# bioinformatics-centre/BayesTyper

Measured on AMD Instinct MI355X. Metric: variant-cluster Gibbs iterations/sec + k-mer matches/sec at 1/2/4/8 MI355X, higher is better.
Workload: dtype f64 log-probabilities over u8 k-mer counts (Gibbs); u64/u8 integer (k-mer matching)

## Files before the change

### bayestyper_amd/csrc/bt_gibbs.hip

```cpp
#ifndef BT_SWEEP_OUTLINE
#define BT_SWEEP_INLINE
#endif
#include "bt_genotypes.hpp"
#include "bt_gibbs_kernel.hpp"
#include "bt_gibbs_timeline.hpp"
#include "bt_internal.hpp"

#include <algorithm>
#include <atomic>
#include <chrono>
#include <cmath>
#include <cstring>
#include <map>
#include <memory>
#include <numeric>

using namespace bt;

namespace bt {
hipError_t launch_gibbs_simple_kernel(unsigned grid, uint32_t lds, hipStream_t st, const TileDesc *tiles, uint8_t *pool, const GParams *P, int op, uint32_t a0, uint32_t a1,
                                      unsigned long long *hist, TraceCfg tr, const uint32_t *tile_list, TimelineDev *tl);
hipError_t prepare_gibbs_simple_kernel(int max_lds);
hipError_t launch_gibbs_hot_kernel(unsigned grid, unsigned block, uint32_t lds, hipStream_t st, const TileDesc *tiles, uint8_t *pool, const GParams *P, int op, uint32_t a0, uint32_t a1,
                                   unsigned long long *hist, TraceCfg tr, const uint32_t *tile_list, TimelineDev *tl);
// ... 818 lines not shown
            BT_HIP(launch_gibbs_hot_kernel(c.pack_wgs, LANES * c.pack_waves, c.pack_lds, st, g->d_tiles, g->d_pool, g->d_params, op, a0, a1, hist, tr, (const uint32_t *)c.d_pack, tl));
        else if (tl)
            hipLaunchKernelGGL(gibbs_kernel_tl, dim3((unsigned)c.tiles.size()), dim3(LANES * c.split), c.lds, st, g->d_tiles, g->d_pool, g->d_params, op, a0, a1, hist, tr,
                               (const uint32_t *)c.d_tiles, tl);
        else
            hipLaunchKernelGGL(gibbs_kernel, dim3((unsigned)c.tiles.size()), dim3(LANES * c.split), c.lds, st, g->d_tiles, g->d_pool, g->d_params, op, a0, a1, hist, tr,
                               (const uint32_t *)c.d_tiles);
        BT_CHECK_LAUNCH();
        if (tl) tl += class_waves(c);
        if (wide && c.num_fill) {
            hipLaunchKernelGGL(nan_fill_kernel, dim3(c.num_fill), dim3(256), 0, st, g->d_pool, (const FillChunk *)c.d_fill);
            BT_CHECK_LAUNCH();
        }
        if (c.stream) BT_HIP(hipEventRecord(c.done, st));
    }
    for (auto &c : g->classes)
        if (c.stream) BT_HIP(hipStreamWaitEvent(g->ctx->stream, c.done, 0));
    g->prefill_armed = wide;
    return BT_OK;
}

inline uint64_t align_up(uint64_t x, uint64_t a) { return (x + a - 1) / a * a; }
inline uint32_t tile_lds_bytes(const TileDesc &d) { return d.lds_all ? d.hot_bytes * d.nvm : d.hot_bytes; }
constexpr uint32_t kBulkSubsetDefault = 1;
constexpr uint32_t kMinTileWidth = 4;
constexpr uint32_t kLightLds = 24576;
const uint32_t kClassLds[] = {16384, 32768, 0xFFFFFFFFu};

const uint32_t kElemSize[A_COUNT] = {
     1,  1,  1,  1,  4,  4,  2,  4,  2,  4,  4,  4,  2,
     1,  4,  4,  4,  2,  4,  4,  4,  4,  4,  4,
     4,  1,
     4,  8,  8,  4,  4,  4,  4,  1,  2,  8,  4,  1,
     4,  4,  4,  4,  4,  4,  8,  4,  8,  2,  8,
     8,  4,  8,  1,  4,  4,  8,  1,  1,  8,  4,  8,  4,  1,  4,  8,  4,
     4,  1,  8,  4,  4,  4,  1,  1,  1,  1,  4,  2,  4,  8,  8,  4,  2,  1,  4,  4,  4,  1,  1,  1,  1,  4,  4};

}

extern "C" {

struct bt_gibbs_source {
    bt_ctx *ctx = nullptr;
    uint32_t S = 0, G = 0, C = 0;
    std::vector<ClusterDims> cd;
    std::vector<GroupDims> gd;
// ... 330 lines not shown
        C = (uint32_t)cd_sel.size();
        cd = cd_sel.data();
        gd = gd_sel.data();
    }
    if (G == 0 || C == 0) return fail("bt_gibbs_create: empty batch");
    BT_HIP(hipSetDevice(ctx->device));
    bt_gibbs *g = new bt_gibbs();
    g->ctx = ctx;
    g->G = G;
    g->C = C;
    g->S = S;
    GParams &P = g->P;
    P.S = S;
    P.seed = params->seed;
    P.num_chains = params->num_chains;
    P.burn_in = params->burn_in;
    P.num_iterations = params->num_iterations;
    P.max_hvk = params->max_haplotype_variant_kmers;
    P.noise_seeding = params->noise_seeding;
    P.rate = (double)params->kmer_subsampling_rate;
    {
        const char *e = getenv("BT_GIBBS_BULK_SUBSET");
        P.bulk_subset = e ? (atoi(e) != 0 ? 1u : 0u) : kBulkSubsetDefault;
    }
    for (uint32_t s = 0; s < S; ++s) P.gender[s] = params->gender[s] ? 1 : 0;

#define BT_TRY(x)                \
    do {                         \
        int _rc = (x);           \
        if (_rc != BT_OK) {      \
            bt_gibbs_destroy(g); \
            return _rc;          \
        }                        \
    } while (0)
#define BT_TRYHIP(x)                                                     \
    do {                                                                 \
        hipError_t _e = (x);                                             \
        if (_e != hipSuccess) {                                          \
            bt_gibbs_destroy(g);                                         \
            return fail(std::string(#x) + ": " + hipGetErrorString(_e)); \
        }                                                                \
    } while (0)

    g->h_A.assign(C, 0);
    g->h_var_off.assign((size_t)C + 1, 0);
    for (uint32_t c = 0; c < C; ++c) g->h_var_off[c + 1] = g->h_var_off[c] + cd[c].V;
// ... 2097 lines not shown
```

### bayestyper_amd/csrc/bt_gibbs_tile.hpp

```cpp
#pragma once
#include "bt_rng_device.hpp"

namespace bt {

constexpr unsigned LANES = 64;
constexpr uint16_t NOHAP = 0xFFFF;
constexpr double BT_LN2 = 0.693147180559945309417232121458176568;
constexpr double BT_DBL_EPS = 2.220446049250313080847263336181640625e-16;
#ifndef BT_LINEAR_DRAW_MIN
#define BT_LINEAR_DRAW_MIN 4u
#endif
#ifndef BT_UC_INVALIDATE_MIN
#define BT_UC_INVALIDATE_MIN 64u
#endif
#ifndef BT_EVAL_BLOCK
#define BT_EVAL_BLOCK 4u
#endif
constexpr uint32_t EVB = BT_EVAL_BLOCK;
#ifdef BT_SINGLE
constexpr bool kSingle = true;
#else
constexpr bool kSingle = false;
#endif
#ifdef BT_PACKED
// ... 121 lines not shown
    uint32_t teams;
    uint32_t sblk;
};
#ifndef BT_EV_CAP
#define BT_EV_CAP 32
#endif
constexpr uint32_t EV_CAP = BT_EV_CAP;
constexpr uint32_t KSC_WAYS = 4;
constexpr uint32_t KSC_NOKEY = 0xFFFEFFFEu;
constexpr uint32_t NOHOT = 0xFFFFFFFFu;
constexpr uint32_t RESIDENT_ALL = 0xFFFFFFFEu;
constexpr uint32_t RESIDENT_NEVER = 0xFFFFFFFDu;

struct GParams {
    uint32_t S, seed, num_chains, burn_in, num_iterations, max_hvk, noise_seeding;
    double rate;
    uint8_t gender[32];
    const double BT_GAS *lut_g;
    const double BT_GAS *lut_n;
    const double BT_GAS *lgamma_int;
    const double BT_GAS *gamma_a2;
    uint32_t lgamma_n, gamma_n;
    uint32_t bulk_subset;
};

extern __shared__ __attribute__((aligned(16))) uint8_t bt_lds_raw[];
__device__ inline uint8_t *lds_block() { return (uint8_t *)bt_lds_raw; }
__device__ inline uint32_t pack_slot() { return blockIdx.x * (blockDim.x >> 6) + (uint32_t)__builtin_amdgcn_readfirstlane((int)(threadIdx.x >> 6)); }

__host__ __device__ constexpr bool hot_core(int a) {
    return a == A_SC || a == A_DIP || a == A_NESTPL || a == A_NESTN || a == A_KSCUPD || a == A_PEND || a == A_PENDDIP || a == A_PENDVALID || a == A_EVN || a == A_FREQ || a == A_LOGF ||
           a == A_OBS || a == A_NZ || a == A_NZLIST || a == A_UNEXT || a == A_ZHDR || a == A_ZBKT || a == A_PHDR || a == A_PBKT || a == A_RING || a == A_FNDSAVED;
}

struct Tile {
    uint8_t BT_GAS *base;
    const TileDesc BT_CAS *d;
    uint32_t lane;
    uint32_t plane;
    uint32_t part, copies;
    uint32_t wsh;
    uint8_t *hot;
    uint32_t lds0;
    uint32_t resident;
    template <typename T>
    __device__ inline SPtrF<T, LANES> harr(int a, uint32_t v, uint32_t len) const {
// ... 314 lines not shown
__device__ inline double count_log_prob(const GParams BT_CAS &P, uint32_t s, uint8_t mult, uint8_t count) {
    if (mult == 0) return P.lut_n[s * 256u + count];
    return P.lut_g[((uint32_t)s * 256u + mult) * 256u + count];
}

__device__ inline uint8_t dip_mult(const Vx &c, uint32_t k, uint16_t h1, uint16_t h2) {
    uint8_t m = 0;
    if (h1 != NOHAP) m = (uint8_t)(m + c.M(k, h1));
    if (h2 != NOHAP) m = (uint8_t)(m + c.M(k, h2));
    return m;
}
__device__ inline uint8_t unique_mult(const Vx &c, uint32_t k, uint16_t h1, uint16_t h2, uint8_t gender) {
    uint8_t m = dip_mult(c, k, h1, h2);
    if (c.has_counts(k)) m = (uint8_t)(m + c.ic(k, gender));
    return m;
}
__device__ inline uint8_t multi_mult(const Vx &c, const GParams BT_CAS &P, uint32_t k, uint16_t h1, uint16_t h2, uint16_t p1, uint16_t p2, uint32_t s) {
    const uint8_t icm = c.ic(k, P.gender[s]);
    if (c.count(k, s) == 0) return (uint8_t)(dip_mult(c, k, h1, h2) + icm);
    const uint8_t shared = c.shared_mult()[(uint32_t)c.shared_idx(k) * P.S + s];
    return (uint8_t)(shared - dip_mult(c, k, p1, p2) + dip_mult(c, k, h1, h2) + icm);
}

__device__ inline void freq_reset(const Vx &c) {
    const double f = 1 / (double)c.H;
    const double lf = bt_log(f);
    SPtrF<uint32_t, LANES> obs = c.obs();
    SPtrF<double, LANES> freq = c.freq(), logf = c.logf();
    SPtrF<uint8_t, LANES> nz = c.nz();
    for (uint32_t h = 0; h < c.H; ++h) {
        obs[h] = 0;
        freq[h] = f;
        logf[h] = lf;
        nz[h] = 1;
    }
    if (c.sc()[SC_IS_SPARSE]) {
        uset_clear(c.plus_set());
        Vx::HSet z = c.zero_set();
        uset_clear(z);
        for (uint32_t h = 0; h < c.H; ++h) uset_insert(z, h);
    }
}

template <class G>
__device__ inline uint32_t sparsity_cover(const Vx &c, G &rng) {
    TPtr<uint8_t> rows = c.cover_rows();
    SPtrF<uint32_t, LANES> obs = c.obs();
    SPtrF<uint16_t, LANES> nzl = c.nzlist();
    const uint32_t Hm = c.d().Hm, H = c.H;
// ... 85 lines not shown
        TPtr<uint32_t> dk = c.dip_keys(), df = c.dip_freq();
        for (uint32_t i = 0; i < d.dip_cap; ++i) dk[i] = 0;
        for (size_t i = 0; i < (uint32_t)d.dip_cap * P.S; ++i) df[i] = 0;
        TPtr<uint32_t> sl = c.sclen();
        for (uint32_t i = 0; i < d.scache_n; ++i) sl[i] = 0;
    }
    c.rng_seed(1, prng_seed);
    uint32_t cover;
    {
        MtRing m = c.rng(1);
        cover = sparsity_cover(c, m);
    }
    c.rng_seed(1, prng_seed);
    c.fnd_saved() = 0;
    sc[SC_FND_AVAIL] = 0;
    sc[SC_IS_SPARSE] = cover > 0 ? 1u : 0u;
    if (cover > 0) {
        const double sp = (double)cover / (double)c.H;
        const double cap = 1 - BT_DBL_EPS * 100;
        c.sparsity() = sp < cap ? sp : cap;
        uset_init(c.zero_set());
        uset_init(c.plus_set());
    }
    freq_reset(c);
    sc[SC_CONSTRUCTED] = 1;
}

__device__ inline uint32_t hashed_slot(const Vx &c, uint32_t key) {
    const uint32_t sub = c.d().cache_entries / c.t.copies;
    return ((key * 2654435761u) & (sub - 1u)) + c.t.part * sub;
}

__device__ inline bool wide_table(const TileDesc BT_CAS &d) { return d.cache_mode == 0 && !d.simple && d.cache_entries > BT_UC_INVALIDATE_MIN && d.hoff[A_UCACHE] == NOHOT; }

__device__ inline void cache_clear(const Vx &c, const GParams BT_CAS &P, bool all_copies_run, bool wide_fill = false) {
    const TileDesc BT_CAS &d = c.d();
    if (wide_fill && !all_copies_run && wide_table(d)) {
        c.sc()[SC_UC_DIRTY] = 0;
    } else if (d.cache_mode == 0) {
        c.sc()[SC_UC_DIRTY] = (!all_copies_run && d.cache_entries > BT_UC_INVALIDATE_MIN) ? 2u : 1u;
    } else if (d.cache_mode == 1) {
        TPtr<uint32_t> tg = c.uctag();
        const uint32_t sub = all_copies_run ? d.cache_entries / c.t.copies : d.cache_entries;
        for (uint32_t i = all_copies_run ? c.t.part * sub : 0u, e = i + sub; i < e; ++i) tg[i] = 0;
    }
    if (!kSingle && d.NMm) {
        SPtrF<uint32_t, LANES> mg = c.mgen();
// ... 172 lines not shown
    sc[SC_NSUB_U] = nsu;
    sc[SC_NSUB_M] = nsm;
    TPtr<uint8_t> smm = c.smm(), oth = c.oth();
    for (uint32_t i = bulk ? c.t.part : 0u, step = bulk ? c.t.copies : 1u; i < nsm * P.S; i += step) {
        smm[i] = 0;
        oth[i] = 0;
    }
    for (uint32_t s = 0; s < P.S; ++s) c.mgen()[s] += 1;
    SPtrF<uint8_t, LANES> upd = c.ksc_upd();
    for (uint32_t s = bulk ? c.t.part : 0u, step = bulk ? c.t.copies : 1u; s < P.S; s += step) {
        upd[s] = 1;
        for (uint32_t e = 0; e < KSC_WAYS; ++e) c.ksc_key(s)[e] = KSC_NOKEY;
        c.ksc_key(s)[KSC_WAYS] = 0;
    }
    if (bulk) copies_sync();
}

__device__ BT_NOINLINE void genotyper_reset(Env env, uint32_t vtx, bool bulk) {
    const Vx c = make_vx(make_tile(env), vtx);
    const GParams BT_CAS &P = env_params(env);
    c.sc()[SC_USE_MULTI] = 0;
    sample_kmer_subset(c, P, bulk);
    cache_clear(c, P, true);
    freq_reset(c);
}

__device__ inline uint32_t dip_index(const Vx &c, uint16_t h1, uint16_t h2) {
    if (h2 == NOHAP) return c.H * (c.H + 1) / 2 + h1;
    return (uint32_t)h1 * c.H - ((uint32_t)h1 * ((uint32_t)h1 - 1u)) / 2u + ((uint32_t)h2 - (uint32_t)h1);
}

__device__ inline double unique_log_prob(const Vx &c, const GParams BT_CAS &P, uint32_t s, uint16_t h1, uint16_t h2, uint32_t nsub_u) {
    const TileDesc BT_CAS &d = c.d();
    const uint32_t idx = dip_index(c, h1, h2);
    uint32_t slot = 0;
    const Vx::UCPtr uc = c.ucache();
    if (d.cache_mode == 0) {
        const double v = uc[(uint32_t)s * d.Dcm + idx];
        if (v == v) return v;
    } else if (d.cache_mode == 1) {
        const uint32_t key = s * d.Dcm + idx + 1u;
        slot = hashed_slot(c, key);
        if (c.uctag()[slot] == key) return uc[slot];
    }
    double acc = 0;
    const uint8_t gender = P.gender[s];
    {
// ... 649 lines not shown
                TPtr<double> pn = c.pend_nest(s);
                same = (double)pn[3] == (double)nn;
                for (uint32_t j = 0; j < 2u; ++j)
                    if (j < nn) {
                        TPtr<double> q = c.nest_stats(s, j);
                        same = same && (double)q[0] == (double)pn[4 * j] && (double)q[1] == (double)pn[4 * j + 1] && (double)q[2] == (double)pn[4 * j + 2];
                    }
            } else
                same = true;
            if (same) {
                c.pend()[s] += 1;
                continue;
            }
        }
#endif
#ifdef BT_COLLECT_OUTLINE
        collect_sample_slow(env, vtx, s);
#else
        collect_sample_body(c, P, s, nsub_u, nsub_m);
#endif
    }
}

__device__ BT_SWEEPFN void sample_diplotypes(Env env, uint32_t vtx, bool collect, uint32_t trace_word, bool tracing, uint32_t *trace_buf) {
    const Vx c = make_vx(make_tile(env), vtx);
    const GParams BT_CAS &P = env_params(env);
    const TPtr<uint32_t> trace_row{(uint32_t BT_GAS *)uniform_ptr(trace_buf), trace_word, 6u};
    SPtrF<uint32_t, LANES> sc = c.sc();
    const uint32_t nsub_u = sc[SC_NSUB_U], nsub_m = kSingle ? 0u : (uint32_t)sc[SC_NSUB_M];
    const bool use_multi = !kSingle && sc[SC_USE_MULTI] != 0, is_sparse = sc[SC_IS_SPARSE] != 0;
    uint32_t hap_count = sc[SC_HAP_COUNT];
    PROF_DECL;
    if (sc[SC_UC_DIRTY] == 2u) {
        const Vx::UCPtr ucl = c.ucache();
        const double nan = __builtin_nan("");
        for (uint32_t i = c.t.part, n = c.d().cache_entries; i < n; i += c.t.copies) ucl[i] = nan;
        if (c.t.copies > 1u) copies_sync();
        sc[SC_UC_DIRTY] = 0;
    } else if (sc[SC_UC_DIRTY]) {
        fill_unique_cache(env, vtx);
        sc[SC_UC_DIRTY] = 0;
    }
    PROF(12);
    MtRing rng = c.rng(0);
    SPtrF<uint16_t, LANES> nzl = c.nzlist();
    SPtrF<double, LANES> logf = c.logf();
    SPtrF<uint16_t, LANES> dip = c.dip();
    uint32_t nnz = 0;
    {
        SPtrF<uint8_t, LANES> nz = c.nz();
        for (uint32_t h = 0; h < c.H; ++h)
            if (nz[h]) nzl[nnz++] = (uint16_t)h;
    }
    PROF(0);
    const uint32_t T = c.t.copies > 1u && c.d().teams > 1u ? c.d().teams : 1u;
    const uint32_t tsz = c.t.copies / T, team = c.t.part / tsz, tpart = c.t.part - team * tsz;
    const uint32_t cw = 64u / c.t.copies, gl = (threadIdx.x & 63u) % cw, tlane0 = gl + team * tsz * cw;
    SPtrF<double, LANES> cum = c.cum() + (team < T ? team : 0u) * (c.d().D2m > 1 ? c.d().D2m : 1);
    for (uint32_t s0 = 0; s0 < P.S; s0 += T) {
      double u01 = 0;
      for (uint32_t j = 0; j < T && s0 + j < P.S; ++j) {
          const double u = rng_canonical(rng);
          if (j == team) u01 = u;
      }
      PROF(24);
      const uint32_t s = s0 + team;
      uint32_t mine = 0xFFFFFFFFu;
      if (team < T && s < P.S) {
        const uint16_t p1 = dip[2 * s], p2 = dip[2 * s + 1];
        const uint8_t ploidy = c.nest_ploidy()[s];
        uint32_t gen = 0;
        if (use_multi && nsub_m) {
            multi_refresh(c, P, s, p1, p2, nsub_m);
            gen = c.mgen()[s];
        }
        PROF(1);
        const uint32_t total = ploidy == 2 ? nnz * (nnz + 1) / 2 : (ploidy == 1 ? nnz : 0u);
        const bool chain_only = total <= BT_LINEAR_DRAW_MIN;
        const bool par = !chain_only && tsz > 1u;
        double lpmax = 0;
        auto eval_candidates = [&]() {
            const bool dipl = ploidy == 2;
            const TileDesc BT_CAS &dd = c.d();
            const Vx::UCPtr uc = c.ucache();
            TPtr<double> mc = c.mcache();
            TPtr<uint32_t> uct = c.uctag(), mct = c.mctag(), mcg = c.mcgen();
            const bool multi = use_multi && nsub_m != 0;
            uint32_t a = 0, b = 0;
            auto advance = [&](uint32_t steps) {
                if (!dipl) {
                    a += steps;
                    return;
                }
                while (steps > 0 && a < nnz) {
                    const uint32_t left = nnz - b;
                    if (steps < left) {
                        b += steps;
                        steps = 0;
                    } else {
                        steps -= left;
                        ++a;
                        b = a;
                    }
                }
// ... 9 lines not shown
                uint32_t utag[EVB], mtag[EVB], mgn[EVB];
#pragma unroll
                for (uint32_t q = 0; q < EVB; ++q) {
                    if (q < nb) {
                        ha[q] = nzl[a];
                        hb[q] = dipl ? (uint16_t)nzl[b] : NOHAP;
                        if (dipl) {
                            if (++b == nnz) {
                                ++a;
                                b = a;
                            }
                        } else
                            ++a;
                        const uint32_t idx = dip_index(c, ha[q], hb[q]);
                        ukey[q] = s * dd.Dcm + idx + 1u;
                        uslot[q] = dd.cache_mode == 0 ? s * dd.Dcm + idx : hashed_slot(c, ukey[q]);
                        uval[q] = dd.cache_mode != 2 ? (double)uc[uslot[q]] : 0.0;
                        utag[q] = dd.cache_mode == 1 ? (uint32_t)uct[uslot[q]] : 0u;
                        if (multi) {
                            mtag[q] = mct[uslot[q]];
                            mgn[q] = mcg[uslot[q]];
                            mval[q] = mc[uslot[q]];
                        }
                        la[q] = logf[ha[q]];
                        lb[q] = dipl ? (double)logf[hb[q]] : 0.0;
                    }
                }
                if (multi) {
                    bool need[EVB], any = false;
#pragma unroll
                    for (uint32_t q = 0; q < EVB; ++q) {
                        need[q] = q < nb && !(mtag[q] == ukey[q] && mgn[q] == gen);
                        any = any || need[q];
                    }
                    if (any) {
                        double fresh[EVB];
                        multi_log_prob_block(c, P, s, ha, hb, need, nsub_m, fresh);
#pragma unroll
                        for (uint32_t q = 0; q < EVB; ++q)
                            if (need[q]) {
                                mval[q] = fresh[q];
                                mct[uslot[q]] = ukey[q];
                                mcg[uslot[q]] = gen;
                                mc[uslot[q]] = fresh[q];
                            }
                    }
                }
                {
                    bool umiss[EVB], any = false;
#pragma unroll
                    for (uint32_t q = 0; q < EVB; ++q) {
                        umiss[q] = q < nb && !((dd.cache_mode == 0 && uval[q] == uval[q]) || (dd.cache_mode == 1 && utag[q] == ukey[q]));
                        any = any || umiss[q];
                    }
                    if (any) {
                        double fresh[EVB];
                        unique_log_prob_block(c, P, s, ha, hb, umiss, nsub_u, fresh);
#pragma unroll
                        for (uint32_t q = 0; q < EVB; ++q)
                            if (umiss[q]) uval[q] = fresh[q];
                    }
                }
#pragma unroll
                for (uint32_t q = 0; q < EVB; ++q) {
                    if (q < nb) {
                        double lp = 0;
                        if (!dipl) lp += la[q];
                        else if (ha[q] == hb[q]) lp += 2 * la[q];
                        else lp += BT_LN2 + la[q] + lb[q];
                        lp += uval[q];
                        if (multi) lp += mval[q];
                        lpmax = lp > lpmax ? lp : lpmax;
                        cum[base + q] = lp;
                    }
                }
                if (par) advance(EVB * (stride_blocks - 1u));
            }
            if (par) {
                const double own = lpmax;
                for (uint32_t m = 0; m < tsz; ++m) {
                    const double o = __shfl(own, (int)(tlane0 + m * cw));
                    lpmax = o > lpmax ? o : lpmax;
                }
                copies_sync();
            }
        };
        auto chain_pick = [&](double u01) -> uint32_t {
            if (total == 0) return 0u;
            double run = cum[0];
            for (uint32_t i = 1; i < total; ++i) {
                run = log_addition((double)cum[i], run);
                cum[i] = run;
            }
            const double u = bt_log(u01) + run;
            uint32_t lo = 0, hi = total;
            while (lo < hi) {
                const uint32_t mid = (lo + hi) >> 1;
                if (u < cum[mid]) hi = mid;
                else lo = mid + 1;
            }
            return lo < total ? lo : total - 1;
        };
        uint32_t pick = 0;
        for (bool exact = chain_only;; exact = true) {
            eval_candidates();
            PROF(2);
            if (exact) {
                if (total == 0) (void)bt_log(u01);
                pick = chain_pick(u01);
                PROF(28);
                break;
            }
            double acc = 0, thr = 0, off = 0;
            uint32_t s0 = 0, s1 = total;
            {
                const uint32_t ncp = tsz, L = (total + ncp - 1u) / ncp;
                const uint32_t i0 = tpart * L < total ? tpart * L : total, i1 = i0 + L < total ? i0 + L : total;
                double run = 0;
                for (uint32_t b0 = i0; b0 < i1; b0 += 8) {
                    double e[8];
#pragma unroll
                    for (uint32_t q = 0; q < 8; ++q) e[q] = b0 + q < i1 ? (double)cum[b0 + q] : 0.0;
#pragma unroll
                    for (uint32_t q = 0; q < 8; ++q)
                        if (b0 + q < i1) e[q] = bt_exp(e[q] - lpmax);
#pragma unroll
                    for (uint32_t q = 0; q < 8; ++q)
                        if (b0 + q < i1) {
                            run += e[q];
                            cum[b0 + q] = run;
                        }
                }
                for (uint32_t m = 0; m < ncp; ++m) acc += __shfl(run, (int)(tlane0 + m * cw));
                thr = u01 * acc;
                uint32_t seg = ncp;
                for (uint32_t m = 0; m < ncp; ++m) {
                    const double tseg = __shfl(run, (int)(tlane0 + m * cw));
                    if (seg == ncp) {
                        if (thr < off + tseg) seg = m;
                        else off += tseg;
                    }
                }
                if (tsz > 1u) copies_sync();
                s0 = seg * L < total ? seg * L : total;
                s1 = s0 + L < total ? s0 + L : total;
            }
            PROF(25);
            uint32_t lo = s0, hi = s1;
            while (lo < hi) {
                const uint32_t mid = (lo + hi) >> 1;
                if (thr < off + (double)cum[mid]) hi = mid;
                else lo = mid + 1;
            }
            const double amax = fabs(lpmax) > 1.0 ? fabs(lpmax) : 1.0;
            double margin = 64.0 * (double)total * amax * BT_DBL_EPS;
            margin = (margin > 1e-6 ? margin : 1e-6) * acc;
            const bool safe = lo < s1 && off + (double)cum[lo] - thr > margin && (lo == 0 || thr - (lo == s0 ? off : off + (double)cum[lo - 1]) > margin);
            PROF(26);
            if (safe) {
                pick = lo;
                break;
            }
            PROF_CNT(14, 1000000);
        }
        uint16_t h1 = NOHAP, h2 = NOHAP;
        if (ploidy == 2) {
            uint32_t a = 0, rem = pick;
            while (rem >= nnz - a) {
                rem -= nnz - a;
                ++a;
            }
            h1 = nzl[a];
            h2 = nzl[a + rem];
        } else if (ploidy == 1) {
            h1 = nzl[pick];
        }
        mine = (uint32_t)h1 | ((uint32_t)h2 << 16);
      }
      if (T > 1u) copies_sync();
      PROF(3);
// ... 61 lines not shown
}

template <class G>
__device__ inline double rng_gamma_count(G &rng, NormalState nd, const GParams BT_CAS &P, uint32_t count) {
    const uint32_t ai = count + 1u;
    const double a1 = (double)ai - 1.0 / 3.0;
    const double a2 = ai < P.gamma_n ? (double)P.gamma_a2[ai] : 1.0 / sqrt(9.0 * a1);
    return a1 * rng_gamma_v(rng, nd, a1, a2) * 1.0;
}

__device__ BT_SWEEPFN void sample_haplotype_frequencies(Env env, uint32_t vtx) {
    const Vx c = make_vx(make_tile(env), vtx);
    const GParams BT_CAS &P = env_params(env);
    const TileDesc BT_CAS &d = c.d();
    SPtrF<uint32_t, LANES> sc = c.sc();
    const uint32_t n_obs = sc[SC_HAP_COUNT];
    PROF_DECL;
    if (n_obs > 0) {
        MtRing rng = c.rng(1);
        const NormalState nd = c.fnd();
        SPtrF<uint32_t, LANES> obs = c.obs();
        SPtrF<double, LANES> freq = c.freq();
        SPtrF<uint8_t, LANES> nz = c.nz();
        if (!sc[SC_IS_SPARSE]) {
            double norm = 0;
            for (uint32_t h = 0; h < c.H; ++h) {
                const double f = rng_gamma_count(rng, nd, P, obs[h]);
                freq[h] = f;
                norm += f;
                obs[h] = 0;
            }
            SPtrF<double, LANES> logf = c.logf();
            for (uint32_t h = 0; h < c.H; ++h) {
                const double f = freq[h] / norm;
                freq[h] = f;
                logf[h] = bt_log(f);
            }
        } else {
            Vx::HSet plus = c.plus_set(), zero = c.zero_set();
            SPtrF<uint32_t, LANES> unext = c.unext();
            const uint32_t plus_size = uset_size(plus);
            uint32_t len;
            TPtr<double> vec = c.simplex();
            const bool cached = d.scache_n && n_obs <= 2 * d.S && plus_size <= d.scache_p;
            const uint32_t ci = cached ? (n_obs - 1) * d.scache_p + (plus_size - 1) : 0u;
            if (cached) vec = c.scache() + (uint32_t)ci * d.scache_len;
            constexpr uint32_t PRE = 4;
            const uint32_t pre = d.scache_len < PRE ? d.scache_len : PRE;
            double head[PRE];
#pragma unroll
            for (uint32_t q = 0; q < PRE; ++q) head[q] = (cached && q < pre) ? (double)vec[q] : 0.0;
            len = cached ? (uint32_t)c.sclen()[ci] : 0u;
            if (len == 0) {
                len = simplex_prob_vector(c, P, vec, n_obs, plus_size);
                if (cached) c.sclen()[ci] = len;
#pragma unroll
                for (uint32_t q = 0; q < PRE; ++q) head[q] = q < len ? (double)vec[q] : 0.0;
            }
            PROF(21);
            const double u = rng_canonical(rng);
// ... 37 lines not shown
                            freq[h + q] = 0;
                            nz[h + q] = 0;
                            obs[h + q] = 0;
                        }
                    }
                }
                for (; h < c.H; ++h) {
                    if (nz[h] == 2) nz[h] = 1;
                    else {
                        freq[h] = 0;
                        nz[h] = 0;
                        obs[h] = 0;
                    }
                }
            }
            SPtrF<uint16_t, LANES> nzl = c.nzlist();
            uint32_t np = 0;
            for (uint32_t e = uset_begin(plus); e != US_NONE; e = unext[e]) nzl[np++] = (uint16_t)e;
            uset_clear(plus);
            for (uint32_t i = 0; i < np; ++i) {
                const uint32_t e = nzl[i];
                const double f = freq[e] / norm;
                freq[e] = f;
                c.logf()[e] = bt_log(f);
                uset_insert(zero, e);
                obs[e] = 0;
            }
        }
        mt_close(rng);
    }
    PROF(7);
    sc[SC_HAP_COUNT] = 0;
}

}
```

### bayestyper_amd/lib.py

```python
import ctypes as C
import os

import numpy as np

_HERE = os.path.dirname(os.path.abspath(__file__))
LIB_PATH = os.environ.get("BTGPU_LIB", os.path.join(_HERE, "libbtgpu.so"))

if not os.path.exists(LIB_PATH):
    raise ImportError(
        f"{LIB_PATH} not found: build the HIP extension first (python -c 'import __graft_entry__ as g; g.build()' "
        "or bayestyper_amd/csrc/build.sh). There is no CPU fallback."
    )

_lib = C.CDLL(LIB_PATH)

u8p, u32p, u64p, i64p, f64p, f32p = (C.POINTER(t) for t in (C.c_uint8, C.c_uint32, C.c_uint64, C.c_int64, C.c_double, C.c_float))
vp = C.c_void_p


def _sig(name, argtypes, restype=C.c_int):
    f = getattr(_lib, name)
    f.argtypes = argtypes
    f.restype = restype
    return f
# ... 662 lines not shown
bt_gibbs_result_sizes = _sig("bt_gibbs_result_sizes", [vp, u64p, u64p])
bt_gibbs_result_fetch = _sig("bt_gibbs_result_fetch", [vp] * 7)
bt_gibbs_result_words = _sig("bt_gibbs_result_words", [vp, C.POINTER(vp), u64p])
bt_gibbs_genotypes = _sig("bt_gibbs_genotypes", [vp, vp, C.POINTER(vp), u64p])
bt_gibbs_trace_enable = _sig("bt_gibbs_trace_enable", [vp, C.c_uint32])
bt_gibbs_trace_fetch = _sig("bt_gibbs_trace_fetch", [vp, vp, C.c_uint64, u64p])
bt_gibbs_posterior_summary = _sig("bt_gibbs_posterior_summary", [vp, vp])
bt_gibbs_timeline_enable = _sig("bt_gibbs_timeline_enable", [vp, C.c_uint32])
bt_gibbs_timeline_sizes = _sig("bt_gibbs_timeline_sizes", [vp, u64p, u32p, u32p, u32p])
bt_gibbs_timeline_fetch = _sig("bt_gibbs_timeline_fetch", [vp, vp, C.c_uint64, u64p])
bt_gibbs_timeline_summary = _sig("bt_gibbs_timeline_summary", [vp, C.c_uint64, C.c_uint32, C.c_uint32, vp])
bt_gibbs_device_bytes = _sig("bt_gibbs_device_bytes", [vp, u64p])
bt_gibbs_source_create = _sig("bt_gibbs_source_create", [vp, C.c_uint32, vp, C.POINTER(vp)])
bt_gibbs_source_create_from_paths = _sig("bt_gibbs_source_create_from_paths", [vp, C.c_uint32, vp, vp, C.POINTER(vp)])
bt_gibbs_source_fetch = _sig("bt_gibbs_source_fetch", [vp, vp, vp])
bt_gibbs_source_destroy = _sig("bt_gibbs_source_destroy", [vp])
bt_gibbs_source_device_bytes = _sig("bt_gibbs_source_device_bytes", [vp, u64p])
bt_gibbs_create_from_source = _sig("bt_gibbs_create_from_source", [vp, vp, vp, vp, C.c_uint32, C.POINTER(vp)])
bt_gibbs_state_bytes = _sig("bt_gibbs_state_bytes", [vp, vp, vp, u64p])
bt_gibbs_state_bytes_from_source = _sig("bt_gibbs_state_bytes_from_source", [vp, vp, vp, C.c_uint32, u64p])
bt_diag_uset_replay = _sig("bt_diag_uset_replay", [C.c_uint32, vp, vp, C.c_uint64, vp, u32p])
bt_diag_rng = _sig("bt_diag_rng", [C.c_uint32, C.c_int, vp, vp, C.c_uint64, vp])
bt_diag_bulk_bernoulli = _sig("bt_diag_bulk_bernoulli", [C.c_uint32, C.c_uint64, C.c_uint32, C.c_double, C.c_uint32, C.c_int, vp, vp, vp])
bt_genotype_text_sizes = _sig("bt_genotype_text_sizes", [vp, vp, C.c_uint64, u64p, u64p])
bt_genotype_text = _sig("bt_genotype_text", [vp, vp, C.c_uint64, vp, C.c_uint64, vp, C.c_uint64, u64p, u64p, u32p])
bt_gibbs_genotype_text = _sig("bt_gibbs_genotype_text", [vp, vp, C.POINTER(vp), u64p, C.POINTER(vp), u64p, u32p])
bt_diag_genotype_text = _sig("bt_diag_genotype_text", [vp, C.c_uint64, vp, C.c_uint64, vp, C.c_uint64, u64p, u64p, u32p])
bt_diag_format_g6 = _sig("bt_diag_format_g6", [vp, C.c_uint64, vp, vp])
bt_diag_genotype_cluster = _sig("bt_diag_genotype_cluster", [C.c_uint32, C.c_uint32, C.c_uint32, vp, vp, vp, C.c_uint64, vp, vp, vp, vp, vp, vp, vp, C.c_uint64, u64p])
bt_diag_kmer_set_order = _sig("bt_diag_kmer_set_order", [vp, C.c_uint32, C.c_uint64, C.c_uint, vp, vp])
bt_diag_kmer_set_order_staged = _sig("bt_diag_kmer_set_order_staged", [vp, C.c_uint32, C.c_uint64, C.c_uint, vp, vp])
bt_kmer_set_orders = _sig("bt_kmer_set_orders", [vp, vp, vp, C.c_uint32, C.c_uint, C.c_uint64, C.c_uint32, vp, vp, vp])
bt_paths_multigroup_info = _sig("bt_paths_multigroup_info", [vp, vp])


TIMELINE_RECORD = np.dtype([("start_tick", np.uint64), ("end_tick", np.uint64), ("hw_id", np.uint32), ("xcc_id", np.uint32), ("tile", np.uint32), ("wave", np.uint32),
                            ("launch", np.uint32), ("launch_class", np.uint16), ("kernel", np.uint8), ("op", np.uint8), ("groups", np.uint32), ("lds_bytes", np.uint32)])
assert TIMELINE_RECORD.itemsize == 48
TIMELINE_KERNELS = ("general", "hot", "simple", "single")
_TIMELINE_SUMMARY_FIELDS = ("records", "unfinished", "first_start", "last_end", "busy_ticks", "peak_live", "median_end", "idle_after_median_ticks", "last_record")


def timeline_summary(records, launch=None, launch_class=None):
    records = np.ascontiguousarray(records, TIMELINE_RECORD)
    out = np.zeros(len(_TIMELINE_SUMMARY_FIELDS), np.uint64)
    check(bt_gibbs_timeline_summary(_np_ptr(records) if len(records) else None, len(records), 0xFFFFFFFF if launch is None else int(launch),
# ... 618 lines not shown
```

### include/btgpu.h

```cpp
#ifndef BTGPU_H
#define BTGPU_H

#include <stddef.h>
#include <stdint.h>

#ifdef __cplusplus
extern "C" {
#endif

#define BT_OK 0
#define BT_ERR 1

typedef struct bt_ctx bt_ctx;

const char *bt_last_error(void);
int bt_version(void);
int bt_device_count(int *count);

int bt_ctx_create(int device_id, bt_ctx **out);
int bt_ctx_clone(bt_ctx *ctx, bt_ctx **out);
int bt_ctx_destroy(bt_ctx *ctx);
int bt_ctx_set_stream(bt_ctx *ctx, void *hip_stream);
int bt_ctx_use_default_stream(bt_ctx *ctx);
int bt_sync(bt_ctx *ctx);
// ... 313 lines not shown
} bt_gibbs_timeline_summary_t;
int bt_gibbs_timeline_enable(bt_gibbs *g, uint32_t max_launches);
int bt_gibbs_timeline_sizes(bt_gibbs *g, uint64_t *records, uint32_t *launches, uint32_t *dropped, uint32_t *tick_khz);
int bt_gibbs_timeline_fetch(bt_gibbs *g, bt_gibbs_timeline_record *h_out, uint64_t capacity, uint64_t *n);
int bt_gibbs_timeline_summary(const bt_gibbs_timeline_record *r, uint64_t n, uint32_t launch, uint32_t launch_class, bt_gibbs_timeline_summary_t *out);

typedef struct bt_noise_rng {
    uint32_t mt[624];
    uint32_t mt_pos;
    uint32_t saved_available;
    double saved;
} bt_noise_rng;
typedef struct bt_noise_model bt_noise_model;
int bt_noise_model_create(bt_ctx *ctx, uint32_t num_samples, const float *h_prior, bt_noise_model **out);
int bt_noise_model_destroy(bt_noise_model *m);
int bt_noise_model_set_rng(bt_noise_model *m, const bt_noise_rng *h_rng);
int bt_noise_model_get_rng(bt_noise_model *m, bt_noise_rng *h_rng);
int bt_gibbs_noise_chain(bt_gibbs *g, bt_noise_model *m, uint32_t num_iterations, uint32_t first_collect,
                         int (*reduce)(void *user, uint64_t *d_hist, uint64_t n), void *user, double *h_rates);

int bt_diag_uset_replay(uint32_t universe, const uint8_t *ops, const uint32_t *values, uint64_t num_ops, uint32_t *h_order, uint32_t *n);
int bt_diag_rng(uint32_t seed, int kind, const double *a, const double *b, uint64_t n, double *h_out);
int bt_diag_bulk_bernoulli(uint32_t seed, uint64_t discard, uint32_t n, double p, uint32_t ring_cap, int ahead, uint8_t *h_flags, uint32_t *h_tail, uint32_t *h_state);
int bt_diag_genotype_cluster(uint32_t S, uint32_t H, uint32_t V, const uint16_t *hap_allele, const uint16_t *var_num_alleles, const uint8_t *var_has_dependency,
                             uint64_t num_diplotypes, const uint16_t *h1, const uint16_t *h2, const uint32_t *freq, const double *stats, const uint8_t *ploidy,
                             const bt_genotype_filters *f, uint32_t *h_words, uint64_t capacity, uint64_t *num_words);
int bt_diag_genotype_text(const uint32_t *h_words, uint64_t num_words, uint8_t *h_text, uint64_t text_capacity, uint32_t *h_index, uint64_t index_capacity, uint64_t *text_bytes,
                          uint64_t *index_words, uint32_t *num_not_covered);
int bt_diag_format_g6(const double *h_values, uint64_t n, char *h_text16, int32_t *h_len);
int bt_diag_kmer_set_order(const uint64_t *h_kmers, uint32_t n, uint64_t initial_buckets, unsigned k, uint32_t *h_rank, uint64_t *h_final_buckets);
int bt_diag_kmer_set_order_staged(const uint64_t *h_kmers, uint32_t n, uint64_t initial_buckets, unsigned k, uint32_t *h_rank, uint64_t *h_final_buckets);

typedef struct bt_deflate_stats {
    uint64_t pieces, stored_pieces;
    uint64_t literals, matches, matched_bytes;
    uint64_t bytes_in, bytes_out;
    double seconds_h2d, seconds_kernels, seconds_d2h, seconds_host;
} bt_deflate_stats;
int bt_deflate_bound(uint64_t n, uint64_t *capacity);
int bt_deflate(bt_ctx *ctx, const uint8_t *d_in, uint64_t n, int last, uint8_t *d_out, uint64_t capacity, uint64_t *h_out_bytes, bt_deflate_stats *stats);
int bt_gzip_save(bt_ctx *ctx, const char *path, const uint8_t *h_data, uint64_t n, uint32_t threads, bt_deflate_stats *stats);
int bt_diag_deflate(const uint8_t *h_in, uint64_t n, int last, uint8_t *h_out, uint64_t capacity, uint64_t *out_bytes, bt_deflate_stats *stats);

int bt_bgzf_bound(uint64_t n, uint64_t *capacity, uint64_t *blocks);
int bt_bgzf(bt_ctx *ctx, const uint8_t *d_in, uint64_t n, int eof, uint8_t *d_out, uint64_t capacity, uint64_t *h_out_bytes, uint64_t *h_block_offsets, bt_deflate_stats *stats);
int bt_bgzf_save(bt_ctx *ctx, const char *path, const uint8_t *h_data, uint64_t n, uint32_t threads, uint64_t *h_block_offsets, uint64_t offsets_capacity, bt_deflate_stats *stats);
// ... 8 lines not shown
```

Before: 1.243 billion.

## Screen diplotype draws with f32 hardware exp2 and lazily computed log-frequencies

Adds a screened draw path, enabled by default: the first pass evaluates candidates without log-frequency terms and builds the cumulative weights as frequency products times a float32 hardware exp2, then accepts the pick only if it lies outside a widened safety margin. Otherwise it falls back to an exact f64 pass, computing logf on demand only for the nonzero haplotypes. This removes the per-update log of every frequency and the f64 exp in the prefix sum. It also lowers the linear-draw threshold to zero so the parallel screened path covers small sets. A host/device diagnostic entry point is added for checking the screen. Risks are more exact-path fallbacks when margins fail, noinline call overhead, and draw-order differences from the lower-precision screening.

```diff
diff --git a/bayestyper_amd/csrc/bt_gibbs.hip b/bayestyper_amd/csrc/bt_gibbs.hip
--- a/bayestyper_amd/csrc/bt_gibbs.hip
+++ b/bayestyper_amd/csrc/bt_gibbs.hip
@@ -864,6 +864,8 @@
 
 inline uint64_t align_up(uint64_t x, uint64_t a) { return (x + a - 1) / a * a; }
 inline uint32_t tile_lds_bytes(const TileDesc &d) { return d.lds_all ? d.hot_bytes * d.nvm : d.hot_bytes; }
+constexpr uint32_t kF32DrawDefault = 1;
+constexpr uint32_t kScreenMinDefault = 0;
 constexpr uint32_t kBulkSubsetDefault = 1;
 constexpr uint32_t kMinTileWidth = 4;
 constexpr uint32_t kLightLds = 24576;
@@ -1240,6 +1242,12 @@
     {
         const char *e = getenv("BT_GIBBS_BULK_SUBSET");
         P.bulk_subset = e ? (atoi(e) != 0 ? 1u : 0u) : kBulkSubsetDefault;
+    }
+    {
+        const char *e = getenv("BT_GIBBS_F32_DRAW");
+        P.f32_draw = e ? (atoi(e) != 0 ? 1u : 0u) : kF32DrawDefault;
+        const char *m = getenv("BT_GIBBS_SCREEN_MIN");
+        P.screen_min = m ? (uint32_t)strtoul(m, nullptr, 0) : kScreenMinDefault;
     }
     for (uint32_t s = 0; s < S; ++s) P.gender[s] = params->gender[s] ? 1 : 0;
 
diff --git a/bayestyper_amd/csrc/bt_gibbs_draw_screen.hip b/bayestyper_amd/csrc/bt_gibbs_draw_screen.hip
--- /dev/null
+++ b/bayestyper_amd/csrc/bt_gibbs_draw_screen.hip
@@ -0,0 +1,133 @@
+#include <string>
+#include <vector>
+#include "../../include/btgpu.h"
+#include "bt_gibbs_draw_screen.hpp"
+#include "bt_internal.hpp"
+
+namespace bt {
+namespace {
+
+struct IdentityIndex {
+    __host__ __device__ inline uint32_t operator[](uint32_t i) const { return i; }
+};
+
+struct ScreenExp2Host {
+    const int8_t *ulps;
+    uint64_t *k;
+    inline float operator()(float r) const {
+        float e = (float)exp2((double)r);
+        if (ulps) {
+            for (int s = ulps[*k]; s > 0; --s) e = nextafterf(e, INFINITY);
+            for (int s = ulps[*k]; s < 0; ++s) e = nextafterf(e, 0.0f);
+        }
+        ++*k;
+        return e;
+    }
+};
+
+template <class X2>
+__host__ __device__ inline void screen_one_set(double *cum, double *e, const double *freq, uint32_t nnz, bool dipl, uint32_t total, double u01, X2 x2_e, X2 x2_draw, uint32_t *pick, uint8_t *safe) {
+    if (total == 0) {
+        *pick = 0;
+        *safe = 0;
+        return;
+    }
+    double xmax = cum[0];
+    for (uint32_t q = 1; q < total; ++q) xmax = cum[q] > xmax ? cum[q] : xmax;
+    for (uint32_t q = 0; q < total; ++q) e[q] = screen_E(cum[q] - xmax, x2_e);
+    double acc;
+    *safe = screen_draw(cum, IdentityIndex(), freq, nnz, dipl, total, xmax, u01, x2_draw, pick, &acc) ? 1 : 0;
+}
+
+__global__ void draw_screen_kernel(uint32_t num_sets, const uint64_t *x_off, double *cum, double *e, const uint64_t *freq_off, const double *freq, const uint32_t *nnz, const uint8_t *ploidy,
+                                   const double *u01, uint32_t *pick, uint8_t *safe) {
+    const uint32_t s = blockIdx.x * blockDim.x + threadIdx.x;
+    if (s >= num_sets) return;
+    const uint64_t x0 = x_off[s];
+    screen_one_set(cum + x0, e + x0, freq + freq_off[s], nnz[s], ploidy[s] == 2, (uint32_t)(x_off[s + 1] - x0), u01[s], ScreenExp2Hw(), ScreenExp2Hw(), pick + s, safe + s);
+}
+
+__global__ void screen_exp_kernel(uint64_t n, const double *x, double *out) {
+    const uint64_t i = (uint64_t)blockIdx.x * blockDim.x + threadIdx.x;
+    if (i < n) out[i] = screen_E(x[i], ScreenExp2Hw());
+}
+
+template <typename T>
+struct DevBuf {
+    T *p = nullptr;
+    ~DevBuf() {
+        if (p) (void)hipFree(p);
+    }
+    hipError_t up(const T *h, size_t n, hipStream_t st) {
+        hipError_t e = hipMalloc((void **)&p, (n ? n : 1) * sizeof(T));
+        if (e == hipSuccess && h && n) e = hipMemcpyAsync(p, h, n * sizeof(T), hipMemcpyHostToDevice, st);
+        return e;
+    }
+    hipError_t down(T *h, size_t n, hipStream_t st) const { return n ? hipMemcpyAsync(h, p, n * sizeof(T), hipMemcpyDeviceToHost, st) : hipSuccess; }
+};
+
+}
+}
+
+using namespace bt;
+
+extern "C" int bt_diag_draw_screen(bt_ctx *ctx, uint32_t num_sets, const uint64_t *x_off, const double *x, const uint64_t *freq_off, const double *freq, const uint32_t *nnz,
+                                   const uint8_t *ploidy, const double *u01, const int8_t *exp_ulps, uint32_t *h_pick, uint8_t *h_safe, double *h_e, uint64_t num_exp, const double *exp_x,
+                                   double *h_exp) {
+    if (num_sets && (!x_off || !x || !freq_off || !freq || !nnz || !ploidy || !u01 || !h_pick || !h_safe || !h_e)) return fail("bt_diag_draw_screen: null argument");
+    if (num_exp && (!exp_x || !h_exp)) return fail("bt_diag_draw_screen: null argument");
+    if (ctx && exp_ulps) return fail("bt_diag_draw_screen: the exponential is perturbed on the host only");
+    for (uint32_t s = 0; s < num_sets; ++s) {
+        const uint64_t total = ploidy[s] == 2 ? (uint64_t)nnz[s] * (nnz[s] + 1ull) / 2 : (ploidy[s] == 1 ? nnz[s] : ~0ull);
+        if (x_off[s + 1] < x_off[s] || x_off[s + 1] - x_off[s] != total || total >> 31 || freq_off[s + 1] < freq_off[s] || freq_off[s + 1] - freq_off[s] != nnz[s] || (s == 0 && (x_off[0] || freq_off[0])))
+            return fail("bt_diag_draw_screen: set " + std::to_string(s) + ": offsets do not match nnz and ploidy (1 or 2)");
+    }
+    const uint64_t nx = num_sets ? x_off[num_sets] : 0, nf = num_sets ? freq_off[num_sets] : 0;
+    if (!ctx) {
+        std::vector<double> cum(x, x + nx);
+        uint64_t k_e = 0, k_draw = 0;
+        for (uint32_t s = 0; s < num_sets; ++s) {
+            const uint64_t x0 = x_off[s];
+            k_e = k_draw = x0;
+            screen_one_set(cum.data() + x0, h_e + x0, freq + freq_off[s], nnz[s], ploidy[s] == 2, (uint32_t)(x_off[s + 1] - x0), u01[s], ScreenExp2Host{exp_ulps, &k_e},
+                           ScreenExp2Host{exp_ulps, &k_draw}, h_pick + s, h_safe + s);
+        }
+        uint64_t k = 0;
+        for (uint64_t i = 0; i < num_exp; ++i) h_exp[i] = screen_E(exp_x[i], ScreenExp2Host{nullptr, &k});
+        return BT_OK;
+    }
+    BT_HIP(hipSetDevice(ctx->device));
+    hipStream_t st = ctx->stream;
+    if (num_sets) {
+        DevBuf<uint64_t> d_xoff, d_foff;
+        DevBuf<double> d_cum, d_e, d_freq, d_u;
+        DevBuf<uint32_t> d_nnz, d_pick;
+        DevBuf<uint8_t> d_pl, d_safe;
+        BT_HIP(d_xoff.up(x_off, (size_t)num_sets + 1, st));
+        BT_HIP(d_foff.up(freq_off, (size_t)num_sets + 1, st));
+        BT_HIP(d_cum.up(x, nx, st));
+        BT_HIP(d_e.up(nullptr, nx, st));
+        BT_HIP(d_freq.up(freq, nf, st));
+        BT_HIP(d_u.up(u01, num_sets, st));
+        BT_HIP(d_nnz.up(nnz, num_sets, st));
+        BT_HIP(d_pl.up(ploidy, num_sets, st));
+        BT_HIP(d_pick.up(nullptr, num_sets, st));
+        BT_HIP(d_safe.up(nullptr, num_sets, st));
+        draw_screen_kernel<<<(num_sets + 63u) / 64u, 64, 0, st>>>(num_sets, d_xoff.p, d_cum.p, d_e.p, d_foff.p, d_freq.p, d_nnz.p, d_pl.p, d_u.p, d_pick.p, d_safe.p);
+        BT_CHECK_LAUNCH();
+        BT_HIP(d_pick.down(h_pick, num_sets, st));
+        BT_HIP(d_safe.down(h_safe, num_sets, st));
+        BT_HIP(d_e.down(h_e, nx, st));
+        BT_HIP(hipStreamSynchronize(st));
+    }
+    if (num_exp) {
+        DevBuf<double> d_x, d_out;
+        BT_HIP(d_x.up(exp_x, num_exp, st));
+        BT_HIP(d_out.up(nullptr, num_exp, st));
+        screen_exp_kernel<<<(unsigned)((num_exp + 255u) / 256u), 256, 0, st>>>(num_exp, d_x.p, d_out.p);
+        BT_CHECK_LAUNCH();
+        BT_HIP(d_out.down(h_exp, num_exp, st));
+        BT_HIP(hipStreamSynchronize(st));
+    }
+    return BT_OK;
+}
diff --git a/bayestyper_amd/csrc/bt_gibbs_draw_screen.hpp b/bayestyper_amd/csrc/bt_gibbs_draw_screen.hpp
--- /dev/null
+++ b/bayestyper_amd/csrc/bt_gibbs_draw_screen.hpp
@@ -0,0 +1,122 @@
+#pragma once
+#include <math.h>
+#include <stdint.h>
+
+#ifndef BT_SCREEN_HD
+#if defined(__HIPCC__) || defined(__CUDACC__)
+#define BT_SCREEN_HD __host__ __device__ inline
+#else
+#define BT_SCREEN_HD inline
+#endif
+#endif
+
+namespace bt {
+
+constexpr double SCREEN_LOG2E = 1.442695040888963407359924681001892137;
+constexpr double SCREEN_DBL_EPS = 2.220446049250313080847263336181640625e-16;
+constexpr double SCREEN_WEIGHT_REL = 1.3e-7;
+constexpr double SCREEN_MARGIN_REL = 16.0 * 2.0 * SCREEN_WEIGHT_REL;
+constexpr double SCREEN_FREQ_MIN = 1e-12;
+constexpr double SCREEN_TOTAL_MIN = 1e-280;
+constexpr double SCREEN_LOGF_SPAN = 56.0;
+
+#if defined(__HIPCC__)
+struct ScreenExp2Hw {
+    __device__ inline float operator()(float r) const { return __builtin_amdgcn_exp2f(r); }
+};
+#endif
+
+template <class X2>
+BT_SCREEN_HD double screen_E(double x, X2 x2) {
+    double y = x * SCREEN_LOG2E;
+    y = y > -1100.0 ? y : -1100.0;
+    const double n = __builtin_rint(y);
+    const float r = (float)(y - n);
+    return __builtin_ldexp((double)x2(r), (int)n);
+}
+
+BT_SCREEN_HD double screen_weight(double fa, double fb, bool twice, double e) { return (twice ? 2.0 : 1.0) * fa * fb * e; }
+
+template <class CumP, class NzlP, class FreqP, class X2>
+BT_SCREEN_HD double screen_prefix(CumP cum, NzlP nzl, FreqP freq, uint32_t nnz, bool dipl, uint32_t i0, uint32_t i1, double xmax, X2 x2) {
+    uint32_t a = i0, b = i0;
+    if (dipl) {
+        uint32_t rem = i0;
+        a = 0;
+        while (a < nnz && rem >= nnz - a) {
+            rem -= nnz - a;
+            ++a;
+        }
+        b = a + rem;
+    }
+    double run = 0;
+    bool tiny = false;
+    for (uint32_t i = i0; i < i1; i += 4) {
+        double x[4], fa[4], fb[4];
+        uint32_t ha[4], hb[4];
+        bool twice[4];
+#pragma unroll
+        for (uint32_t q = 0; q < 4; ++q) {
+            const bool on = i + q < i1;
+            x[q] = on ? (double)cum[i + q] : 0.0;
+            ha[q] = on ? (uint32_t)nzl[a] : 0u;
+            hb[q] = on && dipl ? (uint32_t)nzl[b] : 0u;
+            twice[q] = dipl && a != b;
+            if (on) {
+                if (!dipl) ++a;
+                else if (++b == nnz) {
+                    ++a;
+                    b = a;
+                }
+            }
+        }
+#pragma unroll
+        for (uint32_t q = 0; q < 4; ++q) {
+            fa[q] = (double)freq[ha[q]];
+            fb[q] = dipl ? (double)freq[hb[q]] : 1.0;
+            tiny = tiny || (i + q < i1 && (fa[q] < SCREEN_FREQ_MIN || fb[q] < SCREEN_FREQ_MIN));
+        }
+#pragma unroll
+        for (uint32_t q = 0; q < 4; ++q)
+            if (i + q < i1) {
+                run += screen_weight(fa[q], fb[q], twice[q], screen_E(x[q] - xmax, x2));
+                cum[i + q] = run;
+            }
+    }
+    return tiny ? __builtin_nan("") : run;
+}
+
+template <class CumP>
+BT_SCREEN_HD uint32_t screen_search(CumP cum, uint32_t lo, uint32_t hi, double off, double thr) {
+    while (lo < hi) {
+        const uint32_t mid = (lo + hi) >> 1;
+        if (thr < off + (double)cum[mid]) hi = mid;
+        else lo = mid + 1;
+    }
+    return lo;
+}
+
+BT_SCREEN_HD double screen_margin(uint32_t total, double xmax, double acc) {
+    const double ax = fabs(xmax), amax = (ax > 1.0 ? ax : 1.0) + SCREEN_LOGF_SPAN;
+    double m = 64.0 * (double)total * amax * SCREEN_DBL_EPS;
+    m = m > 1e-6 ? m : 1e-6;
+    m = m > SCREEN_MARGIN_REL ? m : SCREEN_MARGIN_REL;
+    return m * acc;
+}
+
+template <class CumP>
+BT_SCREEN_HD bool screen_safe(CumP cum, uint32_t lo, uint32_t s0, uint32_t s1, double off, double thr, double margin) {
+    return lo < s1 && off + (double)cum[lo] - thr > margin && (lo == 0 || thr - (lo == s0 ? off : off + (double)cum[lo - 1]) > margin);
+}
+
+template <class CumP, class NzlP, class FreqP, class X2>
+BT_SCREEN_HD bool screen_draw(CumP cum, NzlP nzl, FreqP freq, uint32_t nnz, bool dipl, uint32_t total, double xmax, double u01, X2 x2, uint32_t *pick, double *acc_out) {
+    const double acc = screen_prefix(cum, nzl, freq, nnz, dipl, 0u, total, xmax, x2);
+    const double thr = u01 * acc;
+    const uint32_t lo = screen_search(cum, 0u, total, 0.0, thr);
+    *pick = lo < total ? lo : total - 1u;
+    *acc_out = acc;
+    return acc > SCREEN_TOTAL_MIN && screen_safe(cum, lo, 0u, total, 0.0, thr, screen_margin(total, xmax, acc));
+}
+
+}
diff --git a/bayestyper_amd/csrc/bt_gibbs_tile.hpp b/bayestyper_amd/csrc/bt_gibbs_tile.hpp
--- a/bayestyper_amd/csrc/bt_gibbs_tile.hpp
+++ b/bayestyper_amd/csrc/bt_gibbs_tile.hpp
@@ -1,5 +1,6 @@
 #pragma once
 #include "bt_rng_device.hpp"
+#include "bt_gibbs_draw_screen.hpp"
 
 namespace bt {
 
@@ -167,6 +168,8 @@
     const double BT_GAS *gamma_a2;
     uint32_t lgamma_n, gamma_n;
     uint32_t bulk_subset;
+    uint32_t f32_draw;
+    uint32_t screen_min;
 };
 
 extern __shared__ __attribute__((aligned(16))) uint8_t bt_lds_raw[];
@@ -527,9 +530,9 @@
     return (uint8_t)(shared - dip_mult(c, k, p1, p2) + dip_mult(c, k, h1, h2) + icm);
 }
 
-__device__ inline void freq_reset(const Vx &c) {
+__device__ inline void freq_reset(const Vx &c, bool lazy_logf) {
     const double f = 1 / (double)c.H;
-    const double lf = bt_log(f);
+    const double lf = lazy_logf ? 0.0 : bt_log(f);
     SPtrF<uint32_t, LANES> obs = c.obs();
     SPtrF<double, LANES> freq = c.freq(), logf = c.logf();
     SPtrF<uint8_t, LANES> nz = c.nz();
@@ -661,7 +664,7 @@
         uset_init(c.zero_set());
         uset_init(c.plus_set());
     }
-    freq_reset(c);
+    freq_reset(c, P.f32_draw != 0);
     sc[SC_CONSTRUCTED] = 1;
 }
 
@@ -880,7 +883,7 @@
     c.sc()[SC_USE_MULTI] = 0;
     sample_kmer_subset(c, P, bulk);
     cache_clear(c, P, true);
-    freq_reset(c);
+    freq_reset(c, P.f32_draw != 0);
 }
 
 __device__ inline uint32_t dip_index(const Vx &c, uint16_t h1, uint16_t h2) {
@@ -1576,6 +1579,21 @@
     }
 }
 
+__device__ BT_NOINLINE void fill_logf(Env env, uint32_t vtx, uint32_t nnz) {
+    const Vx c = make_vx(make_tile(env), vtx);
+    SPtrF<uint16_t, LANES> nzl = c.nzlist();
+    SPtrF<double, LANES> freq = c.freq(), logf = c.logf();
+    for (uint32_t i = 0; i < nnz; ++i) {
+        const uint32_t h = nzl[i];
+        logf[h] = bt_log((double)freq[h]);
+    }
+}
+
+__device__ BT_NOINLINE double screen_prefix_segment(Env env, uint32_t vtx, uint32_t team, uint32_t nnz, bool dipl, uint32_t i0, uint32_t i1, double xmax) {
+    const Vx c = make_vx(make_tile(env), vtx);
+    return screen_prefix(c.cum() + team * (c.d().D2m > 1 ? c.d().D2m : 1), c.nzlist(), c.freq(), nnz, dipl, i0, i1, xmax, ScreenExp2Hw());
+}
+
 __device__ BT_SWEEPFN void sample_diplotypes(Env env, uint32_t vtx, bool collect, uint32_t trace_word, bool tracing, uint32_t *trace_buf) {
     const Vx c = make_vx(make_tile(env), vtx);
     const GParams BT_CAS &P = env_params(env);
@@ -1601,6 +1619,8 @@
     SPtrF<double, LANES> logf = c.logf();
     SPtrF<uint16_t, LANES> dip = c.dip();
     uint32_t nnz = 0;
+    const bool f32 = P.f32_draw != 0;
+    const uint32_t linear_min = f32 ? P.screen_min : BT_LINEAR_DRAW_MIN;
     {
         SPtrF<uint8_t, LANES> nz = c.nz();
         for (uint32_t h = 0; h < c.H; ++h)
@@ -1630,10 +1650,10 @@
         }
         PROF(1);
         const uint32_t total = ploidy == 2 ? nnz * (nnz + 1) / 2 : (ploidy == 1 ? nnz : 0u);
-        const bool chain_only = total <= BT_LINEAR_DRAW_MIN;
+        const bool chain_only = total <= linear_min;
         const bool par = !chain_only && tsz > 1u;
         double lpmax = 0;
-        auto eval_candidates = [&]() {
+        auto eval_candidates = [&](const bool screen) {
             const bool dipl = ploidy == 2;
             const TileDesc BT_CAS &dd = c.d();
             const Vx::UCPtr uc = c.ucache();
@@ -1689,8 +1709,8 @@
                             mgn[q] = mcg[uslot[q]];
                             mval[q] = mc[uslot[q]];
                         }
-                        la[q] = logf[ha[q]];
-                        lb[q] = dipl ? (double)logf[hb[q]] : 0.0;
+                        la[q] = screen ? 0.0 : (double)logf[ha[q]];
+                        lb[q] = dipl && !screen ? (double)logf[hb[q]] : 0.0;
                     }
                 }
                 if (multi) {
@@ -1732,7 +1752,8 @@
                 for (uint32_t q = 0; q < EVB; ++q) {
                     if (q < nb) {
                         double lp = 0;
-                        if (!dipl) lp += la[q];
+                        if (screen) lp = 0;
+                        else if (!dipl) lp += la[q];
                         else if (ha[q] == hb[q]) lp += 2 * la[q];
                         else lp += BT_LN2 + la[q] + lb[q];
                         lp += uval[q];
@@ -1770,7 +1791,8 @@
         };
         uint32_t pick = 0;
         for (bool exact = chain_only;; exact = true) {
-            eval_candidates();
+            if (exact && f32 && total) fill_logf(env, vtx, nnz);
+            eval_candidates(f32 && !exact);
             PROF(2);
             if (exact) {
                 if (total == 0) (void)bt_log(u01);
@@ -1784,20 +1806,22 @@
                 const uint32_t ncp = tsz, L = (total + ncp - 1u) / ncp;
                 const uint32_t i0 = tpart * L < total ? tpart * L : total, i1 = i0 + L < total ? i0 + L : total;
                 double run = 0;
-                for (uint32_t b0 = i0; b0 < i1; b0 += 8) {
-                    double e[8];
-#pragma unroll
-                    for (uint32_t q = 0; q < 8; ++q) e[q] = b0 + q < i1 ? (double)cum[b0 + q] : 0.0;
-#pragma unroll
-                    for (uint32_t q = 0; q < 8; ++q)
-                        if (b0 + q < i1) e[q] = bt_exp(e[q] - lpmax);
-#pragma unroll
-                    for (uint32_t q = 0; q < 8; ++q)
-                        if (b0 + q < i1) {
-                            run += e[q];
-                            cum[b0 + q] = run;
-                        }
-                }
+                if (f32) run = screen_prefix_segment(env, vtx, team < T ? team : 0u, nnz, ploidy == 2, i0, i1, lpmax);
+                else
+                    for (uint32_t b0 = i0; b0 < i1; b0 += 8) {
+                        double e[8];
+#pragma unroll
+                        for (uint32_t q = 0; q < 8; ++q) e[q] = b0 + q < i1 ? (double)cum[b0 + q] : 0.0;
+#pragma unroll
+                        for (uint32_t q = 0; q < 8; ++q)
+                            if (b0 + q < i1) e[q] = bt_exp(e[q] - lpmax);
+#pragma unroll
+                        for (uint32_t q = 0; q < 8; ++q)
+                            if (b0 + q < i1) {
+                                run += e[q];
+                                cum[b0 + q] = run;
+                            }
+                    }
                 for (uint32_t m = 0; m < ncp; ++m) acc += __shfl(run, (int)(tlane0 + m * cw));
                 thr = u01 * acc;
                 uint32_t seg = ncp;
@@ -1813,16 +1837,15 @@
                 s1 = s0 + L < total ? s0 + L : total;
             }
             PROF(25);
-            uint32_t lo = s0, hi = s1;
-            while (lo < hi) {
-                const uint32_t mid = (lo + hi) >> 1;
-                if (thr < off + (double)cum[mid]) hi = mid;
-                else lo = mid + 1;
-            }
-            const double amax = fabs(lpmax) > 1.0 ? fabs(lpmax) : 1.0;
-            double margin = 64.0 * (double)total * amax * BT_DBL_EPS;
-            margin = (margin > 1e-6 ? margin : 1e-6) * acc;
-            const bool safe = lo < s1 && off + (double)cum[lo] - thr > margin && (lo == 0 || thr - (lo == s0 ? off : off + (double)cum[lo - 1]) > margin);
+            const uint32_t lo = screen_search(cum, s0, s1, off, thr);
+            double margin;
+            if (f32) margin = screen_margin(total, lpmax, acc);
+            else {
+                const double amax = fabs(lpmax) > 1.0 ? fabs(lpmax) : 1.0;
+                margin = 64.0 * (double)total * amax * BT_DBL_EPS;
+                margin = (margin > 1e-6 ? margin : 1e-6) * acc;
+            }
+            const bool safe = (!f32 || acc > SCREEN_TOTAL_MIN) && screen_safe(cum, lo, s0, s1, off, thr, margin);
             PROF(26);
             if (safe) {
                 pick = lo;
@@ -1930,6 +1953,7 @@
         SPtrF<uint32_t, LANES> obs = c.obs();
         SPtrF<double, LANES> freq = c.freq();
         SPtrF<uint8_t, LANES> nz = c.nz();
+        const bool lazy_logf = P.f32_draw != 0;
         if (!sc[SC_IS_SPARSE]) {
             double norm = 0;
             for (uint32_t h = 0; h < c.H; ++h) {
@@ -1939,11 +1963,14 @@
                 obs[h] = 0;
             }
             SPtrF<double, LANES> logf = c.logf();
-            for (uint32_t h = 0; h < c.H; ++h) {
-                const double f = freq[h] / norm;
-                freq[h] = f;
-                logf[h] = bt_log(f);
-            }
+            if (lazy_logf)
+                for (uint32_t h = 0; h < c.H; ++h) freq[h] = freq[h] / norm;
+            else
+                for (uint32_t h = 0; h < c.H; ++h) {
+                    const double f = freq[h] / norm;
+                    freq[h] = f;
+                    logf[h] = bt_log(f);
+                }
         } else {
             Vx::HSet plus = c.plus_set(), zero = c.zero_set();
             SPtrF<uint32_t, LANES> unext = c.unext();
@@ -2027,7 +2054,7 @@
                 const uint32_t e = nzl[i];
                 const double f = freq[e] / norm;
                 freq[e] = f;
-                c.logf()[e] = bt_log(f);
+                if (!lazy_logf) c.logf()[e] = bt_log(f);
                 uset_insert(zero, e);
                 obs[e] = 0;
             }
diff --git a/bayestyper_amd/lib.py b/bayestyper_amd/lib.py
--- a/bayestyper_amd/lib.py
+++ b/bayestyper_amd/lib.py
@@ -708,6 +708,7 @@
 bt_diag_uset_replay = _sig("bt_diag_uset_replay", [C.c_uint32, vp, vp, C.c_uint64, vp, u32p])
 bt_diag_rng = _sig("bt_diag_rng", [C.c_uint32, C.c_int, vp, vp, C.c_uint64, vp])
 bt_diag_bulk_bernoulli = _sig("bt_diag_bulk_bernoulli", [C.c_uint32, C.c_uint64, C.c_uint32, C.c_double, C.c_uint32, C.c_int, vp, vp, vp])
+bt_diag_draw_screen = _sig("bt_diag_draw_screen", [vp, C.c_uint32, vp, vp, vp, vp, vp, vp, vp, vp, vp, vp, vp, C.c_uint64, vp, vp])
 bt_genotype_text_sizes = _sig("bt_genotype_text_sizes", [vp, vp, C.c_uint64, u64p, u64p])
 bt_genotype_text = _sig("bt_genotype_text", [vp, vp, C.c_uint64, vp, C.c_uint64, vp, C.c_uint64, u64p, u64p, u32p])
 bt_gibbs_genotype_text = _sig("bt_gibbs_genotype_text", [vp, vp, C.POINTER(vp), u64p, C.POINTER(vp), u64p, u32p])
diff --git a/include/btgpu.h b/include/btgpu.h
--- a/include/btgpu.h
+++ b/include/btgpu.h
@@ -359,6 +359,9 @@
 int bt_diag_uset_replay(uint32_t universe, const uint8_t *ops, const uint32_t *values, uint64_t num_ops, uint32_t *h_order, uint32_t *n);
 int bt_diag_rng(uint32_t seed, int kind, const double *a, const double *b, uint64_t n, double *h_out);
 int bt_diag_bulk_bernoulli(uint32_t seed, uint64_t discard, uint32_t n, double p, uint32_t ring_cap, int ahead, uint8_t *h_flags, uint32_t *h_tail, uint32_t *h_state);
+int bt_diag_draw_screen(bt_ctx *ctx, uint32_t num_sets, const uint64_t *x_off, const double *x, const uint64_t *freq_off, const double *freq, const uint32_t *nnz,
+                        const uint8_t *ploidy, const double *u01, const int8_t *exp_ulps, uint32_t *h_pick, uint8_t *h_safe, double *h_e, uint64_t num_exp, const double *exp_x,
+                        double *h_exp);
 int bt_diag_genotype_cluster(uint32_t S, uint32_t H, uint32_t V, const uint16_t *hap_allele, const uint16_t *var_num_alleles, const uint8_t *var_has_dependency,
                              uint64_t num_diplotypes, const uint16_t *h1, const uint16_t *h2, const uint32_t *freq, const double *stats, const uint8_t *ploidy,
                              const bt_genotype_filters *f, uint32_t *h_words, uint64_t capacity, uint64_t *num_words);
```

Result: faster. 1.260 billion, median of 5 (+1.4%).
